# flo-stilz/Audio-Key-Estimation

Measured on AMD Instinct MI355X. Metric: clips/s (15 s @ 22.05 kHz), HIP CQT + PitchClassNet forward, higher is better.
Workload: dtype f32 accumulation everywhere; pitch / semitone / layer-0 convolutions: f16 activations x f16 weights (per-channel power-of-two scaled) on MFMA, one product; last layer's pitch-class convolutions and heads: 3-term split-bf16 on MFMA (hi*hi + lo*hi + hi*lo); CQT filter bank: 3-term split-bf16 on MFMA

## Files before the change

### audio-key-estimation_amd/csrc/pcnet.hip

```cpp
#include <algorithm>
#include <cmath>
#include <cstdlib>
#include <cstring>
#include <map>
#include <string>
#include <vector>

#include "common.h"
#include "pcnet_kernels.h"
#include "pcnet_bwd_kernels.h"

using namespace ake_k;

namespace {

constexpr double kBnEps = 1e-5;
constexpr size_t kLdsBudget = 64 * 1024;
constexpr size_t kBfFragsPerConv = 14 * 2 * 64 + 64;

struct TensorSpec {
    std::string name;
    int64_t shape[4];
    int ndim;
};
// ... 1022 lines not shown
                b->g_psix[i] = cv.take<float>(B * d.prev_pc * 36 * Ti);
            }
        }
        if (c.denseblock) {
            for (auto* v : {&b->dn_bott_pc, &b->dn_aff1_pc, &b->dn_aff2_pc, &b->dn_bott_p, &b->dn_aff1_p, &b->dn_aff2_p}) v->assign(L, {});
            size_t gb_pc = 0, gb_p = 0;
            for (int i = 0; i < L; ++i) {
                const int Ti = b->Tl[i];
                const auto& d = n->dims[i];
                for (size_t j = 0; j < n->dense_pc[i].size(); ++j) {
                    const DensePack& dp = n->dense_pc[i][j];
                    b->dn_bott_pc[i].push_back(cv.take<float>(B * dp.c1.cout * 12 * Ti));
                    b->dn_aff1_pc[i].push_back(cv.take<float>(3 * static_cast<size_t>(dp.c1.cin)));
                    b->dn_aff2_pc[i].push_back(cv.take<float>(3 * static_cast<size_t>(dp.c1.cout)));
                    gb_pc = std::max(gb_pc, B * dp.c1.cout * 12 * Ti);
                }
                for (size_t j = 0; i >= 1 && j < n->dense_p[i].size(); ++j) {
                    const DensePack& dp = n->dense_p[i][j];
                    b->dn_bott_p[i].push_back(cv.take<float>(B * dp.c1.cout * P * Ti));
                    b->dn_aff1_p[i].push_back(cv.take<float>(3 * static_cast<size_t>(dp.c1.cin)));
                    b->dn_aff2_p[i].push_back(cv.take<float>(3 * static_cast<size_t>(dp.c1.cout)));
                    gb_p = std::max(gb_p, B * dp.c1.cout * P * Ti);
                }
                (void)d;
            }
            b->dn_gbott_pc = cv.take<float>(gb_pc);
            b->dn_gbott_p = cv.take<float>(gb_p);
        }
        b->g_fold0 = cv.take<float>(B * 12 * frames);
        b->g_pcf = cv.take<float>(B * n->final_ch * 12 * b->Tf);
        b->g_hid = cv.take<float>(hid);
        for (int h = 0; h < 3; ++h) {
            if (h == 2 && !c.genre) break;
            for (int j = 0; j + 1 < c.head_layers; ++j) {
                b->hst[h].push_back(cv.take<float>(hid));
                b->aff_hst[h].push_back(cv.take<float>(3 * 2 * n->final_ch));
            }
            b->g_map[h] = cv.take<float>(B * 12 * b->Tf);
        }
    }
    b->bytes = ake::align_up(cv.off, 256);
    return AKE_OK;
}

enum class L0Form : unsigned char { Generic, FusedValu, FusedMfma };
enum class PStack : unsigned char { Generic, F16x3, F16 };
enum class PcStack : unsigned char { Generic, F16x3, Bf16, Fused };
enum class HeadForm : unsigned char { Generic, Bf16First, Head1, Fused };

struct Layer0Plan {
    L0Form form = L0Form::Generic;
    int RP = 0, RPp = 0;
    size_t lds = 0;
};

struct Route {
    bool frames_major = false;
    Layer0Plan l0;
    bool psix_f16 = false;
    int chunk_clips[2] = {0, 0};
    struct Pitch {
        PStack stack = PStack::Generic;
        unsigned x3_convs = 0;
        struct PerChunk {
            P2pPsPlan first, mid, last;
            P2pStackPlan stack;
            P2pX3Plan x3[2];
        } k[2];
    } p[4];
    PcStack pc = PcStack::Generic;
    unsigned pc_x3_convs = 0;
    HeadForm heads = HeadForm::Generic;
    bool genre_bf = false;
    bool heads_pool = false;
    int heads_mt = 0;
    int T1 = 0, T2 = 0, TpB = 0;
    size_t hf_lds = 0;

    int chunk_kind(int B) const { return B == chunk_clips[0] ? 0 : 1; }
};

Layer0Plan layer0_plan(const ake_pcnet* n, int T0, bool mel16, bool mel_fm) {
    const auto& c = n->cfg;
    const int P = c.pitches, NF = c.n_filters;
    Layer0Plan g;
    if (c.num_layers < 2 || c.resblock || c.denseblock || c.p2pc_conv || c.stay_sixth || NF < 2 || NF > 4 || c.conv_layers < 1 || c.conv_layers > 4 || c.kernel_size != 7 || P % 36 || T0 < 1) return g;
    const PackedConv& sp = n->semi[0];
    if (sp.cin != 1 || sp.co != 1) return g;
    bool mfma = c.precision == AKE_PRECISION_MIXED;
    for (int j = 0; j < c.conv_layers; ++j) {
        const PackedConv& pc = n->pc2pc[0][j];
        if (pc.co != 4 || pc.groups != 1 || pc.kh != 12 || pc.kw != 7 || pc.cout != NF || pc.cin != (j == 0 ? 1 : NF)) return g;
        mfma = mfma && pc.l0_off >= 0;
    }
    if (n->dims[1].prev_pc != NF) return g;
    g.RP = 4 * ((T0 + 3) / 4) + 8;
    g.RPp = (T0 + 8 + 1) / 2 * 2;
    const size_t lds_v = (static_cast<size_t>(9) * 12 * g.RP + static_cast<size_t>(P) * T0) * sizeof(float);
    if (lds_v > 150 * 1024 || (static_cast<long long>(P) * T0) % 4 || !mel16) return g;
    const size_t lds_m = (static_cast<size_t>(4) * 12 * g.RP + static_cast<size_t>(2) * 12 * g.RPp * 4 + static_cast<size_t>(P) * T0) * sizeof(float);
    const bool take_mfma = mfma && lds_m <= 150 * 1024;
    if (mel_fm && (!take_mfma || P % 4)) return g;
    g.form = take_mfma ? L0Form::FusedMfma : L0Form::FusedValu;
    g.lds = take_mfma ? lds_m : lds_v;
    return g;
}

Route build_route(const ake_pcnet* n, bool train, int batch, int chunk, int frames, const float* mel, const void* ws, bool mel_fm) {
    Route r;
    const auto& c = n->cfg;
    const int L = c.num_layers;
    const bool ws16 = !(reinterpret_cast<uintptr_t>(ws) & 15);
    int Tl[4];
    for (int i = 0; i < L; ++i) Tl[i] = i < 2 ? frames : Tl[i - 1] / c.time_pool_size;
    const int Tf = L > 1 ? Tl[L - 1] / c.time_pool_size : frames;
    if (batch < 1 || chunk < 1 || Tf < 1) return r;
    r.chunk_clips[0] = std::min(batch, chunk);
    r.chunk_clips[1] = batch > chunk ? batch % chunk : 0;

    if (!train && L > 1) r.l0 = layer0_plan(n, Tl[0], !(reinterpret_cast<uintptr_t>(mel) & 15), mel_fm);
    if (r.l0.form == L0Form::FusedMfma && !g_keep_taps && !c.pc2p_mem && n->dims[1].prev_p == 1 && p2p_uses_f16(n, 1, Tl[1])) {
        r.psix_f16 = true;
        for (int k = 0; k < 2 && r.psix_f16; ++k)
            if (r.chunk_clips[k])
                r.psix_f16 = p2p_ps_plan(P2pIn::SrcF16x4, 1, n->dims[1].prev_pc, P2pOut::Plane, n->dims[1].out_p, false, r.chunk_clips[k], c.pitches, Tl[1], ws16).ok;
    }

    const int P = c.stay_sixth ? c.pitches / 3 : c.pitches;
    int cp = 1;
    for (int i = 1; i < L && !c.denseblock && !c.resblock; ++i) {
        const LayerDims& d = n->dims[i];
        Route::Pitch& rp = r.p[i];
        const int Ti = Tl[i], c0 = cp, c1 = c.pc2p_mem ? 0 : d.prev_pc;
        if (!train && p2p_uses_f16(n, i, Ti)) {
            rp.stack = PStack::F16;
            const bool semi = p2p_fuses_semi(n, i, P, Ti);
            for (int k = 0; k < 2; ++k) {
                const int B = r.chunk_clips[k];
                if (!B) continue;
                const P2pIn in0 = (i == 1 && r.psix_f16) ? P2pIn::SrcF16x4 : ((mel_fm && i == 1) ? P2pIn::SrcFramesMajor : P2pIn::Src);
                rp.k[k].first = p2p_ps_plan(in0, c0, c1, P2pOut::Plane, d.out_p, false, B, P, Ti, ws16);
                rp.k[k].mid = p2p_ps_plan(P2pIn::Planes, 0, 0, P2pOut::Plane, d.out_p, false, B, P, Ti, ws16);
                P2pPsPlan& last = rp.k[k].last;
                if (semi) last = p2p_ps_plan(P2pIn::Planes, 0, 0, P2pOut::SemiFold, d.prev_pc + d.out_p, true, B, P, Ti, ws16);
                if (semi && !last.ok) last = p2p_ps_plan(P2pIn::Planes, 0, 0, P2pOut::Semi, d.out_p, true, B, P, Ti, ws16);
                if (!last.ok) last = p2p_ps_plan(P2pIn::Planes, 0, 0, P2pOut::Nchw, d.out_p, false, B, P, Ti, ws16);
                if (in0 == P2pIn::SrcF16x4 && semi) rp.k[k].stack = p2p_stack_plan(c.conv_layers, c0, c1, true, B, P, Ti);
            }
        } else if (!c.pc2p_mem && !c.stay_sixth && (train || (c.precision == AKE_PRECISION_F32X3 && !g_keep_taps))) {
            for (int k = 0; k < 2; ++k) {
                const int B = r.chunk_clips[k];
                if (!B) continue;
                rp.k[k].x3[0] = p2p_f16x3_plan(c0, c1, d.out_p, B, P, Ti, ws16);
                rp.k[k].x3[1] = p2p_f16x3_plan(d.out_p, 0, d.out_p, B, P, Ti, ws16);
            }
            for (int j = 0; j < c.conv_layers && j < 32; ++j)
                if ((train ? n->p2p_t[i][j] : n->p2p[i][j]).bf_off >= 0 && rp.k[0].x3[j > 0].ok) rp.x3_convs |= 1u << j;
// ... 1067 lines not shown
    void time_pool(const float* src, const float* in_aff, int B, int C, int H, int Tn, float* dst, int ctot, int coff) {
        const int tp = n->cfg.time_pool_size;
        const long long total = static_cast<long long>(B) * C * H * (Tn / tp);
        launch_flat("time_pool_kernel", time_pool_kernel, s, total, src, in_aff, dst, C, H, Tn, tp, ctot, coff, total);
    }

    int semi_map(int layer, const float* src, int B, int P, int Tn, float* dst, bool raw) {
        const PackedConv& pc = n->semi[layer];
        SemiTrainArgs ta;
        std::memset(&ta, 0, sizeof(ta));
        ta.s = semi_args(n, pc, src, P, Tn, dst);
        ta.out_lrelu = raw ? 0 : 1;
        return launch_semi_conv(pc, ta, P, B);
    }

    int fold_maps(int layer, const float* maps, int C, int S, int B, int Tn, float* dst, int ctot, int coff) {
        if (!n->cfg.p2pc_conv) return run_fold_max("fold_max_kernel", maps, nullptr, C, S, B, Tn, dst, ctot, coff, s);
        const PackedConv& fc = n->foldc[layer];
        const long long total = static_cast<long long>(B) * C * 12 * Tn;
        launch_flat("fold_conv_kernel", fold_conv_kernel, s, total, maps, n->blob_dev + fc.w_off, n->blob_dev + fc.b_off, dst, C, S / 12, Tn, 0,
                    static_cast<long long>(ctot) * 12 * Tn, coff, total);
        return AKE_OK;
    }

    int layer0_fused(const float* mel, int B) {
        const auto& c = n->cfg;
        const int P = c.pitches, T0 = b.Tl[0], NF = c.n_filters;
        const bool take_mfma = r.l0.form == L0Form::FusedMfma;
        AKE_REQUIRE(r.l0.form != L0Form::Generic && r.l0.lds > 0 && !(reinterpret_cast<uintptr_t>(mel) & 15), AKE_ERR_STATE,
                    "pcnet: the route sent layer 0 to its one-launch form, which this call does not qualify for");
        AKE_REQUIRE(!r.frames_major || take_mfma, AKE_ERR_STATE, "pcnet: the route promised the frames-major input to a layer-0 form that cannot read it");
        AKE_REQUIRE(!r.psix_f16 || (take_mfma && b.melh), AKE_ERR_STATE, "pcnet: the route promised the f16 up_sixth map to a layer-0 form that does not write it");
        const PackedConv& sp = n->semi[0];
        const LayerDims& d1 = n->dims[1];
        Layer0Args a;
        std::memset(&a, 0, sizeof(a));
        a.RP = r.l0.RP; a.RPp = r.l0.RPp;
        a.mel = mel; a.sw = n->blob_dev + sp.w_off; a.sb = n->blob_dev + sp.b_off;
        const int ctot1 = d1.prev_pc + d1.out_p;
        for (int j = 0; j < c.conv_layers; ++j) {
            const PackedConv& pc = n->pc2pc[0][j];
            const bool lastj = j == c.conv_layers - 1;
            a.w[j] = n->blob_dev + pc.w_off; a.b[j] = n->blob_dev + pc.b_off;
            if (take_mfma) a.frag[j] = n->bf_frags_dev + pc.l0_off;
            a.dst[j] = lastj ? b.cat[1] : b.pc_out(false, 0, j).p;
            a.dst_clip_stride[j] = static_cast<long long>(lastj ? ctot1 : NF) * 12 * T0;
        }
        a.uw = n->blob_dev + n->up[1].w_off; a.ub = n->blob_dev + n->up[1].b_off;
        a.fold0 = b.fold0; a.psix = b.psix[1];
        a.H = P; a.T = T0; a.NF = NF; a.n_conv = c.conv_layers;
        static ake::DeviceOnce attr_set;
        if (attr_set.need()) {
            AKE_HIP_CHECK(hipFuncSetAttribute(reinterpret_cast<const void*>(layer0_fused_kernel), hipFuncAttributeMaxDynamicSharedMemorySize, 150 * 1024));
            AKE_HIP_CHECK(hipFuncSetAttribute(reinterpret_cast<const void*>(layer0_mfma_kernel), hipFuncAttributeMaxDynamicSharedMemorySize, 150 * 1024));
            attr_set.mark();
        }
        a.mel_fm = r.frames_major ? 1 : 0;
        a.taps = g_keep_taps ? 1 : 0;
        if (r.psix_f16) { a.psix_h = reinterpret_cast<uint2*>(b.psix[1]); a.psix = nullptr; a.melh = b.melh; }
        ake::ProfScope ps("layer0_fused_kernel", s);
        if (take_mfma) hipLaunchKernelGGL(layer0_mfma_kernel, dim3(B), dim3(512), r.l0.lds, s, a);
        else hipLaunchKernelGGL(layer0_fused_kernel, dim3(B), dim3(512), r.l0.lds, s, a);
        return AKE_OK;
    }

    int entry(const float* mel, int B) {
        const auto& c = n->cfg;
        const int L = c.num_layers, P = c.pitches, T0 = b.Tl[0];
        int rc;
        if (r.l0.form != L0Form::Generic) return layer0_fused(mel, B);
        if (c.stay_sixth && L > 1 && train) {
            if ((rc = semi(0, mel, nullptr, B, P, T0, b.fold0, 1, 0, nullptr))) return rc;
        } else if (c.stay_sixth && L > 1) {
            if ((rc = semi_map(0, mel, B, P, T0, b.p0, false))) return rc;
            if ((rc = fold_maps(0, b.p0, 1, P / 3, B, T0, b.fold0, 1, 0))) return rc;
        } else if (c.denseblock) {
            const int g = c.n_filters * c.conv_layers;
            const int ctot1 = L == 1 ? 1 + g : n->dims[1].prev_pc + n->dims[1].out_p + g;
            float* feat = L == 1 ? b.fold0 : b.cat[1];
            if ((rc = semi(0, mel, nullptr, B, P, T0, feat, ctot1, 0, nullptr))) return rc;
            if (L == 1) return AKE_OK;
            if ((rc = dense_stack(0, 1, feat, ctot1, 1, B, 12, T0, b.pca[0], "conv_mfma_kernel/pc2pc0"))) return rc;
            if ((rc = up_sixth(1, feat, static_cast<long long>(ctot1) * 12 * T0, nullptr, B, n->dims[1].prev_pc, T0, b.psix[1], p2pin_up(1)))) return rc;
            return AKE_OK;
        } else if ((rc = semi(0, mel, nullptr, B, P, T0, b.fold0, 1, 0, nullptr))) return rc;
        if (L == 1) return AKE_OK;
        const LayerDims& d1 = n->dims[1];
        const int ctot1 = d1.prev_pc + d1.out_p;
        Slot src{b.fold0, nullptr};
        int cin = 1;
        const std::string m = "model.0.pc2pc.layer.";
        if (c.resblock && train) {
            if ((rc = res_stack_train(n->pc2pc_t[0], m, 1, Src{b.fold0, 1, nullptr, 0, 0}, nullptr, B, 12, T0, b.pcst[0], b.aff_pcst[0], b.cat[1], ctot1,
                                      "conv_mfma_kernel/pc2pc0")))
                return rc;
            identity(b.aff_cat[1], c.n_filters);
        } else if (c.resblock) {
            if ((rc = res_stack(n->pc2pc[0], 1, Src{b.fold0, 1, nullptr, 0, 0}, B, 12, T0, b.pca[0], b.pcb[0], b.cat[1], ctot1, "conv_mfma_kernel/pc2pc0"))) return rc;
        }
        for (int j = 0; j < c.conv_layers && !c.resblock; ++j) {
            const bool lastj = j == c.conv_layers - 1;
            const Slot dst = lastj ? b.cat_slot(train, 1) : b.pc_out(train, 0, j);
            if ((rc = conv(n->pc2pc[0][j], train ? n->pc2pc_t[0][j] : n->pc2pc[0][j], m + std::to_string(3 * j + 1), 1,
                           Src{src.p, cin, nullptr, 0, 0}, src.aff, B, 12, T0, true, dst.p, lastj ? ctot1 : c.n_filters, 0, dst.aff,
                           "conv_mfma_kernel/pc2pc0")))
                return rc;
            src = dst; cin = c.n_filters;
        }
        if (c.stay_sixth) return AKE_OK;
        if (train) identity(b.aff_p2pin[1], d1.prev_p);
// ... 669 lines not shown
```

### audio-key-estimation_amd/csrc/pcnet_kernels.h

```cpp
#pragma once

#include <hip/hip_runtime.h>

#include "common.h"

namespace ake_k {

constexpr int TW = 4;
constexpr float kSlope = 0.01f;

struct ConvArgs {
    const float* src0;
    const float* src1;
    long long src0_clip_stride, src1_clip_stride;
    int c0, c1, h1;
    int H;
    int T_in;
    int T_out;
    int H_out;
    int py;
    int pad_l;
    int time_circ;
    const float* w;
    const float* bias;
// ... 2141 lines not shown
    if (ks == 0 && qq == 0 && tau == 0) reinterpret_cast<float*>(out + kP2pFragScale)[co] = 1.f / sc;
    unsigned int hi[4] = {0, 0, 0, 0}, lo[4] = {0, 0, 0, 0};
    for (int ci = 0; ci < 8; ++ci) {
        float v = 0.f;
        if (dx >= 0 && dx < 7 && ci < n_in && co < n_out) v = sc * wv(co, ci, dy, dx);
        const _Float16 hv = static_cast<_Float16>(v);
        const unsigned int hb = __builtin_bit_cast(unsigned short, hv);
        const unsigned int lb = f16_bits((v - static_cast<float>(hv)) * kP2pLoScale);
        hi[ci >> 1] |= hb << (16 * (ci & 1));
        lo[ci >> 1] |= lb << (16 * (ci & 1));
    }
    out[(2 * ks + 0) * 64 + lane] = make_uint4(hi[0], hi[1], hi[2], hi[3]);
    out[(2 * ks + 1) * 64 + lane] = make_uint4(lo[0], lo[1], lo[2], lo[3]);
}
__global__ void pack_p2p_f16_raw_jobs_kernel(P2pRawJobs js) {
    const P2pRawJob& J = js.j[blockIdx.y];
    pack_p2p_f16_raw_body(J.w, J.out, J.cin_fwd, J.cout_fwd, J.transpose_flip, blockIdx.x);
}

__global__ void fold_max_kernel(const float* __restrict__ smap, const float* __restrict__ aff, int C, int S, int T, float* __restrict__ dst,
                                long long dst_clip_stride, int dst_coff, long long total) {
    const long long i = static_cast<long long>(blockIdx.x) * blockDim.x + threadIdx.x;
    if (i >= total) return;
    const int t = static_cast<int>(i % T);
    long long r = i / T;
    const int p = static_cast<int>(r % 12); r /= 12;
    const int c = static_cast<int>(r % C);
    const long long clip = r / C;
    const float* src = smap + ((clip * C + c) * S + p) * T + t;
    float best = -INFINITY;
    for (int o = 0; o < S / 12; ++o) best = fmaxf(best, affine_act(src[static_cast<long long>(12 * o) * T], aff, c));
    dst[clip * dst_clip_stride + (static_cast<long long>(dst_coff + c) * 12 + p) * T + t] = best;
}

struct Layer0Args {
    const float* mel;
    const float* sw;
    const float* sb;
    const float* w[4];
    const float* b[4];
    float* dst[4];
    long long dst_clip_stride[4];
    const float* uw;
    const float* ub;
    float* fold0;
    float* psix;
    int H, T, RP, NF, n_conv;
    const uint4* frag[4];
    int taps;
    int RPp;
    int mel_fm;
    uint2* psix_h;
    unsigned int* melh;
};

__global__ __launch_bounds__(512) void layer0_fused_kernel(Layer0Args a) {
    extern __shared__ __attribute__((aligned(16))) float l0[];
    const int clip = blockIdx.x, tid = threadIdx.x;
    const int T = a.T, RP = a.RP, NF = a.NF;
    float* const f0 = l0;
    float* const actA = l0 + 12 * RP;
    float* const actB = actA + 4 * 12 * RP;
    for (int i = tid; i < 9 * 12 * RP; i += 512) l0[i] = 0.f;
    __syncthreads();
    {
        float* const ml = actB + 4 * 12 * RP;
        const float4* mel4 = reinterpret_cast<const float4*>(a.mel + static_cast<long long>(clip) * a.H * T);
        const int n4 = a.H * T / 4;
        for (int i = tid; i < n4; i += 512) reinterpret_cast<float4*>(ml)[i] = mel4[i];
        __syncthreads();
        float w9[9];
#pragma unroll
        for (int i = 0; i < 9; ++i) w9[i] = a.sw[i];
        const float sb = a.sb[0];
        const int n_oct = a.H / 36;
        for (int i = tid; i < 12 * T; i += 512) {
            const int p = i / T, t = i - p * T;
            const int tm = t == 0 ? T - 1 : t - 1, tp = t == T - 1 ? 0 : t + 1;
            float best = -INFINITY;
            for (int o = 0; o < n_oct; ++o) {
                const float* r = ml + 3 * (p + 12 * o) * T;
                float acc = 0.f;
#pragma unroll
                for (int dy = 0; dy < 3; ++dy) {
                    acc = fmaf(r[dy * T + tm], w9[dy * 3 + 0], acc);
                    acc = fmaf(r[dy * T + t], w9[dy * 3 + 1], acc);
                    acc = fmaf(r[dy * T + tp], w9[dy * 3 + 2], acc);
                }
                float v = acc + sb;
                v = v > 0.f ? v : v * kSlope;
                best = fmaxf(best, v);
            }
            f0[p * RP + 3 + t] = best;
            a.fold0[(static_cast<long long>(clip) * 12 + p) * T + t] = best;
        }
    }
    __syncthreads();
    const int nst = (T + 3) / 4;
    const int cp = __builtin_amdgcn_readfirstlane(tid >> 8);
    const int item = tid & 255;
    const float* in = f0;
    float* out = actA;
    int cin = 1;
    for (int j = 0; j < a.n_conv; ++j) {
        typedef const float __attribute__((address_space(4))) cfloat;
        cfloat* w = (cfloat*)(a.w[j] + 2 * cp);
// ... 71 lines not shown
    }
}

struct LocalPoolArgs {
    const float* maps[3];
    float* outs[3];
    int Tm, Tq, W, batch;
};

__global__ void local_pool_kernel(LocalPoolArgs a) {
    const int which = blockIdx.y;
    if (!a.maps[which]) return;
    const int rows = which == 2 ? 11 : 12;
    const int To = which == 2 ? a.Tm : a.Tq;
    const long long i = static_cast<long long>(blockIdx.x) * blockDim.x + threadIdx.x;
    if (i >= static_cast<long long>(a.batch) * rows * To) return;
    const int t = static_cast<int>(i % To);
    const long long row = i / To;
    const float* m = a.maps[which] + row * a.Tm + t;
    float v = m[0];
    if (which < 2) {
        for (int w = 1; w < a.W; ++w) v = fmaxf(v, m[w]);
        if (which == 0) v = 1.f / (1.f + expf(-v));
    }
    a.outs[which][i] = v;
}

__global__ void pack_l0_f16_kernel(const float* __restrict__ w, uint4* __restrict__ out, int cin, int cout) {
    __shared__ int smax[4];
    channel_absmax4(w, cin * 84, smax);
    const int i = blockIdx.x * blockDim.x + threadIdx.x;
    if (i >= 12 * 64) return;
    const int dy = i / 64, lane = i - dy * 64;
    const int n = lane & 15, qq = lane >> 4;
    const int tau = n >> 2, co = n & 3;
    const float sc = f16_weight_scale(__int_as_float(smax[co]));
    if (dy == 0 && qq == 0 && tau == 0) reinterpret_cast<float*>(out + 24 * 64)[co] = 1.f / sc;
    unsigned int hi[4] = {0, 0, 0, 0}, lo[4] = {0, 0, 0, 0};
    for (int e = 0; e < 8; ++e) {
        const int pos = 2 * qq + (e >> 2), ci = e & 3;
        const int dx = pos - tau;
        float v = 0.f;
        if (n < 8 && dx >= 0 && dx < 7 && ci < cin && co < cout) v = sc * w[((ci * 12 + dy) * 7 + dx) * 4 + co];
        const _Float16 hv = static_cast<_Float16>(v);
        const unsigned int hb = __builtin_bit_cast(unsigned short, hv);
        const unsigned int lb = f16_bits((v - static_cast<float>(hv)) * kP2pLoScale);
        hi[e >> 1] |= hb << (16 * (e & 1));
        lo[e >> 1] |= lb << (16 * (e & 1));
    }
    out[(2 * dy + 0) * 64 + lane] = make_uint4(hi[0], hi[1], hi[2], hi[3]);
    out[(2 * dy + 1) * 64 + lane] = make_uint4(lo[0], lo[1], lo[2], lo[3]);
}

__global__ __launch_bounds__(512) void layer0_mfma_kernel(Layer0Args a) {
    extern __shared__ __attribute__((aligned(16))) float l0[];
    const int clip = blockIdx.x, tid = threadIdx.x;
    const int lane = tid & 63, wave = __builtin_amdgcn_readfirstlane(tid >> 6);
    const int r16 = lane & 15, q = lane >> 4;
    const int T = a.T, RP = a.RP, RPp = a.RPp, NF = a.NF;
    f16_saturate_mode();
    float* const fmap = l0;
    unsigned short* const mapA = reinterpret_cast<unsigned short*>(l0 + 4 * 12 * RP);
    const int plane = 12 * RPp * 4;
    unsigned short* const mapB = mapA + 2 * plane;
    float* const ml = reinterpret_cast<float*>(mapB + 2 * plane);
    for (int i = tid; i < 4 * 12 * RP + 2 * plane; i += 512) l0[i] = 0.f;
    {
        const float4* mel4 = reinterpret_cast<const float4*>(a.mel + static_cast<long long>(clip) * a.H * T);
        const int n4 = a.H * T / 4;
        if (a.mel_fm) {
            const int h4 = a.H / 4;
            for (int i = tid; i < n4; i += 512) {
                const int t = i / h4, r4 = (i - t * h4) * 4;
                const float4 v = mel4[i];
                ml[(r4 + 0) * T + t] = v.x; ml[(r4 + 1) * T + t] = v.y; ml[(r4 + 2) * T + t] = v.z; ml[(r4 + 3) * T + t] = v.w;
            }
        } else
            for (int i = tid; i < n4; i += 512) reinterpret_cast<float4*>(ml)[i] = mel4[i];
        __syncthreads();
        if (a.melh) {
            uint4* const mh = reinterpret_cast<uint4*>(a.melh + static_cast<long long>(clip) * a.H * T);
            auto word = [](float v) {
                const _Float16 h = static_cast<_Float16>(v);
                return static_cast<unsigned int>(__builtin_bit_cast(unsigned short, h)) | (f16_bits(v - static_cast<float>(h)) << 16);
            };
            for (int i = tid; i < n4; i += 512) {
                const float4 v = reinterpret_cast<const float4*>(ml)[i];
                mh[i] = make_uint4(word(v.x), word(v.y), word(v.z), word(v.w));
            }
        }
        float w9[9];
#pragma unroll
        for (int i = 0; i < 9; ++i) w9[i] = a.sw[i];
        const float sb = a.sb[0];
        const int n_oct = a.H / 36;
        for (int i = tid; i < 12 * T; i += 512) {
            const int p = i / T, t = i - p * T;
            const int tm = t == 0 ? T - 1 : t - 1, tp = t == T - 1 ? 0 : t + 1;
            float best = -INFINITY;
            for (int o = 0; o < n_oct; ++o) {
                const float* r = ml + 3 * (p + 12 * o) * T;
                float acc = 0.f;
#pragma unroll
                for (int dy = 0; dy < 3; ++dy) {
                    acc = fmaf(r[dy * T + tm], w9[dy * 3 + 0], acc);
                    acc = fmaf(r[dy * T + t], w9[dy * 3 + 1], acc);
                    acc = fmaf(r[dy * T + tp], w9[dy * 3 + 2], acc);
                }
                float v = acc + sb;
                v = v > 0.f ? v : v * kSlope;
                best = fmaxf(best, v);
            }
            const _Float16 bh16 = static_cast<_Float16>(best);
            mapA[(p * RPp + 3 + t) * 4] = __builtin_bit_cast(unsigned short, bh16);
            mapA[12 * RPp * 4 + (p * RPp + 3 + t) * 4] = static_cast<unsigned short>(f16_bits((best - static_cast<float>(bh16)) * kP2pLoScale));
            a.fold0[(static_cast<long long>(clip) * 12 + p) * T + t] = best;
        }
    }
    __syncthreads();
    const int J = (T + 1) / 2, M = 12 * J, n_tiles = (M + 15) / 16;
    const int tau = (r16 >> 2) & 1, co = r16 & 3;
    const unsigned short* in = mapA;
    unsigned short* out = mapB;
    uint4 breg[12], bregl[12], bnext[12], bnextl[12];
    auto frags_of = [&](int j) { return j == 0 ? a.frag[0] : j == 1 ? a.frag[1] : j == 2 ? a.frag[2] : a.frag[3]; };
#pragma unroll
    for (int i = 0; i < 12; ++i) {
        bnext[i] = a.n_conv > 0 ? frags_of(0)[2 * i * 64 + lane] : make_uint4(0, 0, 0, 0);
        bnextl[i] = a.n_conv > 0 ? frags_of(0)[(2 * i + 1) * 64 + lane] : make_uint4(0, 0, 0, 0);
    }
    for (int j = 0; j < a.n_conv; ++j) {
#pragma unroll
        for (int i = 0; i < 12; ++i) { breg[i] = bnext[i]; bregl[i] = bnextl[i]; }
        const float bias = (r16 < 8 && co < NF) ? a.b[j][co] : 0.f;
        const float iscale = reinterpret_cast<const float*>(frags_of(j) + 24 * 64)[co];
        const bool write_dst = a.taps || j == a.n_conv - 1;
        float* const g = a.dst[j] + clip * a.dst_clip_stride[j];
        if (j + 1 < a.n_conv) {
#pragma unroll
            for (int i = 0; i < 12; ++i) { bnext[i] = frags_of(j + 1)[2 * i * 64 + lane]; bnextl[i] = frags_of(j + 1)[(2 * i + 1) * 64 + lane]; }
        }
        for (int tile = wave; tile < n_tiles; tile += 8) {
            int m = tile * 16 + r16;
            m = m < M ? m : M - 1;
            const int p = m / J, jj = m - p * J;
            f32x4c acc = {0.f, 0.f, 0.f, 0.f}, accl = {0.f, 0.f, 0.f, 0.f};
#pragma unroll
            for (int dy = 0; dy < 12; ++dy) {
                int row = p + dy;
                row -= row >= 12 ? 12 : 0;
                const int pos = row * RPp + 2 * jj + 2 * q;
                const f16x8c ah = __builtin_bit_cast(f16x8c, *reinterpret_cast<const uint4*>(in + pos * 4));
                const f16x8c al = __builtin_bit_cast(f16x8c, *reinterpret_cast<const uint4*>(in + plane + pos * 4));
                const f16x8c bh = __builtin_bit_cast(f16x8c, breg[dy]), bl = __builtin_bit_cast(f16x8c, bregl[dy]);
                acc = __builtin_amdgcn_mfma_f32_16x16x32_f16(ah, bh, acc, 0, 0, 0);
                accl = __builtin_amdgcn_mfma_f32_16x16x32_f16(al, bh, accl, 0, 0, 0);
                accl = __builtin_amdgcn_mfma_f32_16x16x32_f16(ah, bl, accl, 0, 0, 0);
            }
            if (r16 < 8 && co < NF) {
#pragma unroll
                for (int i = 0; i < 4; ++i) {
                    const int mm = tile * 16 + 4 * q + i;
                    const int pp = mm / J, t = 2 * (mm - pp * J) + tau;
                    if (mm < M && t < T) {
                        float v = fmaf(fmaf(accl[i], kP2pLoInv, acc[i]), iscale, bias);
                        v = fmaxf(v, v * kSlope);
                        const _Float16 hv = static_cast<_Float16>(v);
                        out[(pp * RPp + 3 + t) * 4 + co] = __builtin_bit_cast(unsigned short, hv);
                        out[plane + (pp * RPp + 3 + t) * 4 + co] = static_cast<unsigned short>(f16_bits((v - static_cast<float>(hv)) * kP2pLoScale));
                        fmap[(co * 12 + pp) * RP + 3 + t] = v;
                        if (write_dst) g[(static_cast<long long>(co) * 12 + pp) * T + t] = v;
                    }
                }
            }
        }
        __syncthreads();
        const unsigned short* tmp = in;
        in = out;
        out = const_cast<unsigned short*>(tmp);
    }
    if (a.psix_h) {
        typedef const float __attribute__((address_space(4))) cfloat;
        cfloat* uw = (cfloat*)a.uw;
        cfloat* ub = (cfloat*)a.ub;
        uint2* ph = a.psix_h + static_cast<long long>(clip) * 36 * T;
        for (int i = tid; i < 12 * T; i += 512) {
            const int p = i / T, t = i - p * T;
            float x[4];
#pragma unroll
            for (int ci = 0; ci < 4; ++ci) x[ci] = fmap[(ci * 12 + p) * RP + 3 + t];
#pragma unroll
            for (int jj = 0; jj < 3; ++jj) {
                unsigned int h[4];
#pragma unroll
                for (int co2 = 0; co2 < 4; ++co2) {
                    float acc = co2 < NF ? ub[co2 < NF ? co2 : 0] : 0.f;
#pragma unroll
                    for (int ci = 0; ci < 4; ++ci)
                        if (ci < NF && co2 < NF) acc = fmaf(x[ci], uw[(ci * NF + co2) * 3 + jj], acc);
                    acc = acc > 0.f ? acc : acc * kSlope;
                    h[co2] = __builtin_bit_cast(unsigned short, static_cast<_Float16>(acc));
                }
                ph[(3 * p + jj) * T + t] = make_uint2(h[0] | (h[1] << 16), h[2] | (h[3] << 16));
            }
        }
    } else if (a.psix) {
        typedef const float __attribute__((address_space(4))) cfloat;
        cfloat* uw = (cfloat*)a.uw;
        cfloat* ub = (cfloat*)a.ub;
        float* ps = a.psix + static_cast<long long>(clip) * NF * 36 * T;
        for (int i = tid; i < 12 * T; i += 512) {
            const int p = i / T, t = i - p * T;
            float x[4];
#pragma unroll
            for (int ci = 0; ci < 4; ++ci) x[ci] = fmap[(ci * 12 + p) * RP + 3 + t];
            for (int co2 = 0; co2 < NF; ++co2) {
#pragma unroll
                for (int jj = 0; jj < 3; ++jj) {
                    float acc = ub[co2];
#pragma unroll
                    for (int ci = 0; ci < 4; ++ci)
                        if (ci < NF) acc = fmaf(x[ci], uw[(ci * NF + co2) * 3 + jj], acc);
                    ps[(static_cast<long long>(co2) * 36 + 3 * p + jj) * T + t] = acc > 0.f ? acc : acc * kSlope;
                }
            }
        }
    }
}

__global__ void pc2p_mem_kernel(const float* __restrict__ p, const float* __restrict__ psix, float* __restrict__ out, int cp, int ratio, int P, int T,
                                long long total, const float* __restrict__ psix_aff) {
    const long long i = static_cast<long long>(blockIdx.x) * blockDim.x + threadIdx.x;
    if (i >= total) return;
    const int t = static_cast<int>(i % T);
    long long q = i / T;
    const int r = static_cast<int>(q % P);
    q /= P;
    const int c = static_cast<int>(q % cp);
    const long long clip = q / cp;
    const int k = r / (P / 36);
    const float* s = psix + (((clip * cp + c) * ratio) * 36 + k) * T + t;
    float acc = p[i];
    for (int g = 0; g < ratio; ++g) {
        float v = s[static_cast<long long>(g) * 36 * T];
        if (psix_aff) {
            const float* a3 = psix_aff + 3 * (c * ratio + g);
            const float y = fmaf(v, a3[0], a3[1]);
            v = y > 0.f ? y : y * a3[2];
        }
        acc += v;
    }
    out[i] = acc;
}

__global__ void fold_conv_kernel(const float* __restrict__ src, const float* __restrict__ w, const float* __restrict__ bias, float* __restrict__ dst,
                                 int C, int n_oct, int T, int in_lrelu, long long dst_clip_stride, int dst_coff, long long total) {
    const long long i = static_cast<long long>(blockIdx.x) * blockDim.x + threadIdx.x;
    if (i >= total) return;
// ... 236 lines not shown
```

Baseline: 451,200.

## Restructure layer-0 MFMA kernel: tiled mel image, LDS-staged fragments, prefetched A loads

Reworks the fused layer-0 MFMA kernel. The frames-major mel input is stored as a 4x4-transposed tiled image in LDS, with unrolled batched global loads. Next-layer weight fragments are DMA'd into LDS (double-buffered) instead of held in prefetch registers. A-operand loads run a few rows ahead of the MFMAs behind sched barriers, and index math becomes incremental. LDS per block grows to 160 KB, and a specialised NF=4 upsample path keeps weights in registers, adding register pressure and layout complexity.

```diff
diff --git a/audio-key-estimation_amd/csrc/pcnet.hip b/audio-key-estimation_amd/csrc/pcnet.hip
--- a/audio-key-estimation_amd/csrc/pcnet.hip
+++ b/audio-key-estimation_amd/csrc/pcnet.hip
@@ -1098,6 +1098,9 @@
     L0Form form = L0Form::Generic;
     int RP = 0, RPp = 0;
     size_t lds = 0;
+    bool tiled = false;
+    int img_sq = 0, img_sb = 0, img_sr = 0;
+    bool frag_lds = false;
 };
 
 struct Route {
@@ -1126,6 +1129,7 @@
     int chunk_kind(int B) const { return B == chunk_clips[0] ? 0 : 1; }
 };
 
+constexpr size_t kL0MaxLds = 160 * 1024;
 Layer0Plan layer0_plan(const ake_pcnet* n, int T0, bool mel16, bool mel_fm) {
     const auto& c = n->cfg;
     const int P = c.pitches, NF = c.n_filters;
@@ -1149,6 +1153,19 @@
     if (mel_fm && (!take_mfma || P % 4)) return g;
     g.form = take_mfma ? L0Form::FusedMfma : L0Form::FusedValu;
     g.lds = take_mfma ? lds_m : lds_v;
+    if (take_mfma) {
+        const size_t maps = lds_m - static_cast<size_t>(P) * T0 * sizeof(float);
+        const size_t frag_bytes = c.conv_layers > 1 ? static_cast<size_t>(2) * 24 * 64 * sizeof(uint4) : 0;
+        const int sq = 4 * P + ((36 - (4 * P & 31)) & 31);
+        const size_t tiled_bytes = static_cast<size_t>((T0 + 3) / 4) * sq * sizeof(float);
+        g.tiled = mel_fm && maps + tiled_bytes <= kL0MaxLds;
+        g.img_sq = g.tiled ? sq : 4;
+        g.img_sb = g.tiled ? P : T0;
+        g.img_sr = g.tiled ? 4 : 4 * T0;
+        const size_t img_bytes = g.tiled ? tiled_bytes : static_cast<size_t>(P) * T0 * sizeof(float);
+        g.frag_lds = frag_bytes && maps + std::max(img_bytes, frag_bytes) <= kL0MaxLds;
+        g.lds = maps + (g.frag_lds ? std::max(img_bytes, frag_bytes) : img_bytes);
+    }
     return g;
 }
 
@@ -2322,10 +2339,14 @@
         static ake::DeviceOnce attr_set;
         if (attr_set.need()) {
             AKE_HIP_CHECK(hipFuncSetAttribute(reinterpret_cast<const void*>(layer0_fused_kernel), hipFuncAttributeMaxDynamicSharedMemorySize, 150 * 1024));
-            AKE_HIP_CHECK(hipFuncSetAttribute(reinterpret_cast<const void*>(layer0_mfma_kernel), hipFuncAttributeMaxDynamicSharedMemorySize, 150 * 1024));
+            AKE_HIP_CHECK(hipFuncSetAttribute(reinterpret_cast<const void*>(layer0_mfma_kernel), hipFuncAttributeMaxDynamicSharedMemorySize, static_cast<int>(kL0MaxLds)));
             attr_set.mark();
         }
         a.mel_fm = r.frames_major ? 1 : 0;
+        a.frag_lds = r.l0.frag_lds ? 1 : 0;
+        a.img_tiled = r.l0.tiled ? 1 : 0; a.img_sq = r.l0.img_sq; a.img_sb = r.l0.img_sb; a.img_sr = r.l0.img_sr;
+        AKE_REQUIRE(!r.l0.tiled || r.frames_major, AKE_ERR_STATE, "pcnet: layer 0's image was planned for a frames-major input that the route refused");
+        AKE_REQUIRE(r.l0.lds <= kL0MaxLds, AKE_ERR_STATE, "pcnet: layer 0's one-launch form does not fit the LDS at this shape");
         a.taps = g_keep_taps ? 1 : 0;
         if (r.psix_f16) { a.psix_h = reinterpret_cast<uint2*>(b.psix[1]); a.psix = nullptr; a.melh = b.melh; }
         ake::ProfScope ps("layer0_fused_kernel", s);
diff --git a/audio-key-estimation_amd/csrc/pcnet_kernels.h b/audio-key-estimation_amd/csrc/pcnet_kernels.h
--- a/audio-key-estimation_amd/csrc/pcnet_kernels.h
+++ b/audio-key-estimation_amd/csrc/pcnet_kernels.h
@@ -2217,6 +2217,9 @@
     int mel_fm;
     uint2* psix_h;
     unsigned int* melh;
+    int img_tiled;
+    int frag_lds;
+    int img_sq, img_sb, img_sr;
 };
 
 __global__ __launch_bounds__(512) void layer0_fused_kernel(Layer0Args a) {
@@ -2394,6 +2397,54 @@
     out[(2 * dy + 1) * 64 + lane] = make_uint4(lo[0], lo[1], lo[2], lo[3]);
 }
 
+__device__ __forceinline__ void l0_step(int& qv, int& rv, const int dq, const int dr, const int n) {
+    qv += dq;
+    rv += dr;
+    if (rv >= n) { rv -= n; ++qv; }
+}
+
+template <int NFC>
+__device__ __forceinline__ void l0_up_sixth_h(const Layer0Args& a, const float* fmap, uint2* ph, const int tid) {
+    typedef const float __attribute__((address_space(4))) cfloat;
+    cfloat* uw = (cfloat*)a.uw;
+    cfloat* ub = (cfloat*)a.ub;
+    const int T = a.T, RP = a.RP, NF = NFC ? NFC : a.NF;
+    float wk[NFC ? 48 : 1], bk[NFC ? 4 : 1];
+    if (NFC) {
+#pragma unroll
+        for (int i = 0; i < (NFC ? 48 : 1); ++i) wk[i] = uw[i];
+#pragma unroll
+        for (int i = 0; i < (NFC ? 4 : 1); ++i) bk[i] = ub[i];
+    }
+    for (int i = tid; i < 12 * T; i += 512) {
+        const int p = i / T, t = i - p * T;
+        float x[4];
+#pragma unroll
+        for (int ci = 0; ci < 4; ++ci) x[ci] = fmap[(ci * 12 + p) * RP + 3 + t];
+#pragma unroll
+        for (int jj = 0; jj < 3; ++jj) {
+            unsigned int h[4];
+#pragma unroll
+            for (int co2 = 0; co2 < 4; ++co2) {
+                float acc;
+                if (NFC) {
+                    acc = bk[co2];
+#pragma unroll
+                    for (int ci = 0; ci < 4; ++ci) acc = fmaf(x[ci], wk[(ci * 4 + co2) * 3 + jj], acc);
+                } else {
+                    acc = co2 < NF ? ub[co2 < NF ? co2 : 0] : 0.f;
+#pragma unroll
+                    for (int ci = 0; ci < 4; ++ci)
+                        if (ci < NF && co2 < NF) acc = fmaf(x[ci], uw[(ci * NF + co2) * 3 + jj], acc);
+                }
+                acc = acc > 0.f ? acc : acc * kSlope;
+                h[co2] = __builtin_bit_cast(unsigned short, static_cast<_Float16>(acc));
+            }
+            ph[(3 * p + jj) * T + t] = make_uint2(h[0] | (h[1] << 16), h[2] | (h[3] << 16));
+        }
+    }
+}
+
 __global__ __launch_bounds__(512) void layer0_mfma_kernel(Layer0Args a) {
     extern __shared__ __attribute__((aligned(16))) float l0[];
     const int clip = blockIdx.x, tid = threadIdx.x;
@@ -2406,19 +2457,66 @@
     const int plane = 12 * RPp * 4;
     unsigned short* const mapB = mapA + 2 * plane;
     float* const ml = reinterpret_cast<float*>(mapB + 2 * plane);
-    for (int i = tid; i < 4 * 12 * RP + 2 * plane; i += 512) l0[i] = 0.f;
+    auto frags_of = [&](int j) { return j == 0 ? a.frag[0] : j == 1 ? a.frag[1] : j == 2 ? a.frag[2] : a.frag[3]; };
+    uint4 breg[12], bregl[12];
+#pragma unroll
+    for (int i = 0; i < 12; ++i) {
+        breg[i] = a.n_conv > 0 ? frags_of(0)[2 * i * 64 + lane] : make_uint4(0, 0, 0, 0);
+        bregl[i] = a.n_conv > 0 ? frags_of(0)[(2 * i + 1) * 64 + lane] : make_uint4(0, 0, 0, 0);
+    }
+    const int tau = (r16 >> 2) & 1, co = r16 & 3;
+    float bias_j[4], iscale_j[4];
+#pragma unroll
+    for (int j = 0; j < 4; ++j) {
+        bias_j[j] = (j < a.n_conv && r16 < 8 && co < NF) ? a.b[j][co] : 0.f;
+        iscale_j[j] = j < a.n_conv ? reinterpret_cast<const float*>(a.frag[j] + 24 * 64)[co] : 0.f;
+    }
+    for (int i = tid; i < plane / 2; i += 512) reinterpret_cast<uint4*>(mapA)[i] = make_uint4(0, 0, 0, 0);
     {
         const float4* mel4 = reinterpret_cast<const float4*>(a.mel + static_cast<long long>(clip) * a.H * T);
         const int n4 = a.H * T / 4;
+        const int Sq = a.img_sq, Sb = a.img_sb, Sr = a.img_sr;
+        auto img = [&](int r, int t) { return (t >> 2) * Sq + (t & 3) + (r & 3) * Sb + (r >> 2) * Sr; };
         if (a.mel_fm) {
             const int h4 = a.H / 4;
-            for (int i = tid; i < n4; i += 512) {
+            const int nq = a.img_tiled ? T >> 2 : 0;
+            const int nit = nq * h4;
+            const int sq_i = 512 / h4, sr_i = 512 - sq_i * h4;
+            int fq_i = tid / h4, R_i = tid - fq_i * h4;
+            for (int i0 = tid; i0 < nit; i0 += 512 * 3) {
+                float4 v[3][4];
+                int fqs[3], Rs[3];
+#pragma unroll
+                for (int u = 0; u < 3; ++u) {
+                    const bool live = i0 + 512 * u < nit;
+                    fqs[u] = live ? fq_i : 0; Rs[u] = live ? R_i : 0;
+                    l0_step(fq_i, R_i, sq_i, sr_i, h4);
+#pragma unroll
+                    for (int k = 0; k < 4; ++k) v[u][k] = mel4[(4 * fqs[u] + k) * h4 + Rs[u]];
+                }
+#pragma unroll
+                for (int u = 0; u < 3; ++u) {
+                    float* const d = ml + fqs[u] * Sq + Rs[u] * 4;
+                    *reinterpret_cast<float4*>(d) = make_float4(v[u][0].x, v[u][1].x, v[u][2].x, v[u][3].x);
+                    *reinterpret_cast<float4*>(d + Sb) = make_float4(v[u][0].y, v[u][1].y, v[u][2].y, v[u][3].y);
+                    *reinterpret_cast<float4*>(d + 2 * Sb) = make_float4(v[u][0].z, v[u][1].z, v[u][2].z, v[u][3].z);
+                    *reinterpret_cast<float4*>(d + 3 * Sb) = make_float4(v[u][0].w, v[u][1].w, v[u][2].w, v[u][3].w);
+                }
+            }
+            for (int i = 4 * nit + tid; i < n4; i += 512) {
                 const int t = i / h4, r4 = (i - t * h4) * 4;
                 const float4 v = mel4[i];
-                ml[(r4 + 0) * T + t] = v.x; ml[(r4 + 1) * T + t] = v.y; ml[(r4 + 2) * T + t] = v.z; ml[(r4 + 3) * T + t] = v.w;
-            }
-        } else
-            for (int i = tid; i < n4; i += 512) reinterpret_cast<float4*>(ml)[i] = mel4[i];
+                ml[img(r4 + 0, t)] = v.x; ml[img(r4 + 1, t)] = v.y; ml[img(r4 + 2, t)] = v.z; ml[img(r4 + 3, t)] = v.w;
+            }
+        } else {
+            for (int i0 = tid; i0 < n4; i0 += 512 * 8) {
+                float4 v[8];
+#pragma unroll
+                for (int u = 0; u < 8; ++u) v[u] = mel4[i0 + 512 * u < n4 ? i0 + 512 * u : n4 - 1];
+#pragma unroll
+                for (int u = 0; u < 8; ++u) reinterpret_cast<float4*>(ml)[i0 + 512 * u < n4 ? i0 + 512 * u : n4 - 1] = v[u];
+            }
+        }
         __syncthreads();
         if (a.melh) {
             uint4* const mh = reinterpret_cast<uint4*>(a.melh + static_cast<long long>(clip) * a.H * T);
@@ -2426,9 +2524,26 @@
                 const _Float16 h = static_cast<_Float16>(v);
                 return static_cast<unsigned int>(__builtin_bit_cast(unsigned short, h)) | (f16_bits(v - static_cast<float>(h)) << 16);
             };
-            for (int i = tid; i < n4; i += 512) {
-                const float4 v = reinterpret_cast<const float4*>(ml)[i];
-                mh[i] = make_uint4(word(v.x), word(v.y), word(v.z), word(v.w));
+            auto words = [&](const float4 v) { return make_uint4(word(v.x), word(v.y), word(v.z), word(v.w)); };
+            if (!a.img_tiled) {
+                for (int i = tid; i < n4; i += 512) mh[i] = words(reinterpret_cast<const float4*>(ml)[i]);
+            } else if (!(T & 3)) {
+                const int tq4 = T >> 2, sq_m = 512 / tq4, sr_m = 512 - sq_m * tq4;
+                int r = tid / tq4, tq = tid - r * tq4;
+                for (int i = tid; i < n4; i += 512) {
+                    mh[i] = words(*reinterpret_cast<const float4*>(ml + img(r, 4 * tq)));
+                    l0_step(r, tq, sq_m, sr_m, tq4);
+                }
+            } else {
+                for (int i = tid; i < n4; i += 512) {
+                    float e[4];
+#pragma unroll
+                    for (int k = 0; k < 4; ++k) {
+                        const int r = (4 * i + k) / T;
+                        e[k] = ml[img(r, 4 * i + k - r * T)];
+                    }
+                    mh[i] = words(make_float4(e[0], e[1], e[2], e[3]));
+                }
             }
         }
         float w9[9];
@@ -2439,15 +2554,19 @@
         for (int i = tid; i < 12 * T; i += 512) {
             const int p = i / T, t = i - p * T;
             const int tm = t == 0 ? T - 1 : t - 1, tp = t == T - 1 ? 0 : t + 1;
+            const int fm = (tm >> 2) * Sq + (tm & 3), f0 = (t >> 2) * Sq + (t & 3), fp = (tp >> 2) * Sq + (tp & 3);
+            int ro[3];
+#pragma unroll
+            for (int dy = 0; dy < 3; ++dy) ro[dy] = ((3 * p + dy) & 3) * Sb + ((3 * p + dy) >> 2) * Sr;
             float best = -INFINITY;
             for (int o = 0; o < n_oct; ++o) {
-                const float* r = ml + 3 * (p + 12 * o) * T;
+                const float* r = ml + 9 * o * Sr;
                 float acc = 0.f;
 #pragma unroll
                 for (int dy = 0; dy < 3; ++dy) {
-                    acc = fmaf(r[dy * T + tm], w9[dy * 3 + 0], acc);
-                    acc = fmaf(r[dy * T + t], w9[dy * 3 + 1], acc);
-                    acc = fmaf(r[dy * T + tp], w9[dy * 3 + 2], acc);
+                    acc = fmaf(r[ro[dy] + fm], w9[dy * 3 + 0], acc);
+                    acc = fmaf(r[ro[dy] + f0], w9[dy * 3 + 1], acc);
+                    acc = fmaf(r[ro[dy] + fp], w9[dy * 3 + 2], acc);
                 }
                 float v = acc + sb;
                 v = v > 0.f ? v : v * kSlope;
@@ -2461,91 +2580,88 @@
     }
     __syncthreads();
     const int J = (T + 1) / 2, M = 12 * J, n_tiles = (M + 15) / 16;
-    const int tau = (r16 >> 2) & 1, co = r16 & 3;
+    const int sq_t = 128 / J, sr_t = 128 - sq_t * J, rowE = RPp * 4;
     const unsigned short* in = mapA;
     unsigned short* out = mapB;
-    uint4 breg[12], bregl[12], bnext[12], bnextl[12];
-    auto frags_of = [&](int j) { return j == 0 ? a.frag[0] : j == 1 ? a.frag[1] : j == 2 ? a.frag[2] : a.frag[3]; };
-#pragma unroll
-    for (int i = 0; i < 12; ++i) {
-        bnext[i] = a.n_conv > 0 ? frags_of(0)[2 * i * 64 + lane] : make_uint4(0, 0, 0, 0);
-        bnextl[i] = a.n_conv > 0 ? frags_of(0)[(2 * i + 1) * 64 + lane] : make_uint4(0, 0, 0, 0);
-    }
+    uint4* const fr0 = reinterpret_cast<uint4*>(ml);
     for (int j = 0; j < a.n_conv; ++j) {
-#pragma unroll
-        for (int i = 0; i < 12; ++i) { breg[i] = bnext[i]; bregl[i] = bnextl[i]; }
-        const float bias = (r16 < 8 && co < NF) ? a.b[j][co] : 0.f;
-        const float iscale = reinterpret_cast<const float*>(frags_of(j) + 24 * 64)[co];
+        if (j > 0 && a.frag_lds) {
+            const uint4* fr = fr0 + (j & 1) * 24 * 64;
+#pragma unroll
+            for (int i = 0; i < 12; ++i) { breg[i] = fr[2 * i * 64 + lane]; bregl[i] = fr[(2 * i + 1) * 64 + lane]; }
+        } else if (j > 0) {
+            const uint4* fr = frags_of(j);
+#pragma unroll
+            for (int i = 0; i < 12; ++i) { breg[i] = fr[2 * i * 64 + lane]; bregl[i] = fr[(2 * i + 1) * 64 + lane]; }
+        }
+        const float bias = j == 0 ? bias_j[0] : j == 1 ? bias_j[1] : j == 2 ? bias_j[2] : bias_j[3];
+        const float iscale = j == 0 ? iscale_j[0] : j == 1 ? iscale_j[1] : j == 2 ? iscale_j[2] : iscale_j[3];
         const bool write_dst = a.taps || j == a.n_conv - 1;
         float* const g = a.dst[j] + clip * a.dst_clip_stride[j];
-        if (j + 1 < a.n_conv) {
-#pragma unroll
-            for (int i = 0; i < 12; ++i) { bnext[i] = frags_of(j + 1)[2 * i * 64 + lane]; bnextl[i] = frags_of(j + 1)[(2 * i + 1) * 64 + lane]; }
-        }
+        if (j + 1 < a.n_conv && a.frag_lds) {
+            const uint4* src = frags_of(j + 1);
+            uint4* const dstl = fr0 + ((j + 1) & 1) * 24 * 64;
+#pragma unroll
+            for (int k = 0; k < 3; ++k) {
+                const int c = wave + 8 * k;
+                ake::lds_dma_16(src + c * 64 + lane, static_cast<unsigned int>(reinterpret_cast<unsigned long long>(dstl + c * 64)));
+            }
+        }
+        int pa = (wave * 16 + r16) / J, ja = wave * 16 + r16 - pa * J;
+        int pe = (wave * 16 + 4 * q) / J, je = wave * 16 + 4 * q - pe * J;
         for (int tile = wave; tile < n_tiles; tile += 8) {
-            int m = tile * 16 + r16;
-            m = m < M ? m : M - 1;
-            const int p = m / J, jj = m - p * J;
+            const int p = pa < 12 ? pa : 11, jj = pa < 12 ? ja : J - 1;
             f32x4c acc = {0.f, 0.f, 0.f, 0.f}, accl = {0.f, 0.f, 0.f, 0.f};
+            constexpr int kL0Ahead = 3;
+            f16x8c ah[12], al[12];
+            const int e0 = (p * RPp + 2 * jj + 2 * q) * 4;
+            auto request = [&](int dy) {
+                const int e = e0 + dy * rowE - (dy >= 12 - p ? 12 * rowE : 0);
+                ah[dy] = __builtin_bit_cast(f16x8c, *reinterpret_cast<const uint4*>(in + e));
+                al[dy] = __builtin_bit_cast(f16x8c, *reinterpret_cast<const uint4*>(in + plane + e));
+            };
+#pragma unroll
+            for (int dy = 0; dy < kL0Ahead; ++dy) request(dy);
 #pragma unroll
             for (int dy = 0; dy < 12; ++dy) {
-                int row = p + dy;
-                row -= row >= 12 ? 12 : 0;
-                const int pos = row * RPp + 2 * jj + 2 * q;
-                const f16x8c ah = __builtin_bit_cast(f16x8c, *reinterpret_cast<const uint4*>(in + pos * 4));
-                const f16x8c al = __builtin_bit_cast(f16x8c, *reinterpret_cast<const uint4*>(in + plane + pos * 4));
+                if (dy + kL0Ahead < 12) request(dy + kL0Ahead);
+                __builtin_amdgcn_sched_barrier(0);
                 const f16x8c bh = __builtin_bit_cast(f16x8c, breg[dy]), bl = __builtin_bit_cast(f16x8c, bregl[dy]);
-                acc = __builtin_amdgcn_mfma_f32_16x16x32_f16(ah, bh, acc, 0, 0, 0);
-                accl = __builtin_amdgcn_mfma_f32_16x16x32_f16(al, bh, accl, 0, 0, 0);
-                accl = __builtin_amdgcn_mfma_f32_16x16x32_f16(ah, bl, accl, 0, 0, 0);
+                acc = __builtin_amdgcn_mfma_f32_16x16x32_f16(ah[dy], bh, acc, 0, 0, 0);
+                accl = __builtin_amdgcn_mfma_f32_16x16x32_f16(al[dy], bh, accl, 0, 0, 0);
+                accl = __builtin_amdgcn_mfma_f32_16x16x32_f16(ah[dy], bl, accl, 0, 0, 0);
+                __builtin_amdgcn_sched_barrier(0);
             }
             if (r16 < 8 && co < NF) {
+                int pp = pe, jm = je;
 #pragma unroll
                 for (int i = 0; i < 4; ++i) {
-                    const int mm = tile * 16 + 4 * q + i;
-                    const int pp = mm / J, t = 2 * (mm - pp * J) + tau;
-                    if (mm < M && t < T) {
+                    const int t = 2 * jm + tau;
+                    if (pp < 12 && t < T) {
                         float v = fmaf(fmaf(accl[i], kP2pLoInv, acc[i]), iscale, bias);
                         v = fmaxf(v, v * kSlope);
                         const _Float16 hv = static_cast<_Float16>(v);
                         out[(pp * RPp + 3 + t) * 4 + co] = __builtin_bit_cast(unsigned short, hv);
                         out[plane + (pp * RPp + 3 + t) * 4 + co] = static_cast<unsigned short>(f16_bits((v - static_cast<float>(hv)) * kP2pLoScale));
                         fmap[(co * 12 + pp) * RP + 3 + t] = v;
-                        if (write_dst) g[(static_cast<long long>(co) * 12 + pp) * T + t] = v;
+                        if (write_dst) g[(co * 12 + pp) * T + t] = v;
                     }
+                    l0_step(pp, jm, 0, 1, J);
                 }
             }
-        }
+            l0_step(pa, ja, sq_t, sr_t, J);
+            l0_step(pe, je, sq_t, sr_t, J);
+        }
+        if (j + 1 < a.n_conv && a.frag_lds) __builtin_amdgcn_s_waitcnt(0x0F70);
         __syncthreads();
         const unsigned short* tmp = in;
         in = out;
         out = const_cast<unsigned short*>(tmp);
     }
     if (a.psix_h) {
-        typedef const float __attribute__((address_space(4))) cfloat;
-        cfloat* uw = (cfloat*)a.uw;
-        cfloat* ub = (cfloat*)a.ub;
         uint2* ph = a.psix_h + static_cast<long long>(clip) * 36 * T;
-        for (int i = tid; i < 12 * T; i += 512) {
-            const int p = i / T, t = i - p * T;
-            float x[4];
-#pragma unroll
-            for (int ci = 0; ci < 4; ++ci) x[ci] = fmap[(ci * 12 + p) * RP + 3 + t];
-#pragma unroll
-            for (int jj = 0; jj < 3; ++jj) {
-                unsigned int h[4];
-#pragma unroll
-                for (int co2 = 0; co2 < 4; ++co2) {
-                    float acc = co2 < NF ? ub[co2 < NF ? co2 : 0] : 0.f;
-#pragma unroll
-                    for (int ci = 0; ci < 4; ++ci)
-                        if (ci < NF && co2 < NF) acc = fmaf(x[ci], uw[(ci * NF + co2) * 3 + jj], acc);
-                    acc = acc > 0.f ? acc : acc * kSlope;
-                    h[co2] = __builtin_bit_cast(unsigned short, static_cast<_Float16>(acc));
-                }
-                ph[(3 * p + jj) * T + t] = make_uint2(h[0] | (h[1] << 16), h[2] | (h[3] << 16));
-            }
-        }
+        if (NF == 4) l0_up_sixth_h<4>(a, fmap, ph, tid);
+        else l0_up_sixth_h<0>(a, fmap, ph, tid);
     } else if (a.psix) {
         typedef const float __attribute__((address_space(4))) cfloat;
         cfloat* uw = (cfloat*)a.uw;
```

Result: faster. 462,600 (median of 6 runs) (+2.5%).
